# ana-kuznetsova/Policy-Gradient-ASR

Hardware: AMD Instinct MI355X
Metric: utterances/sec (B=32,T=1000,F=80) policy-grad step, 1/2/4/8 MI355X (higher is better)
Workload: dtype f32 (fp32-faithful: fp32 storage and accumulate; every big product -- recurrent sweeps, W_ih projections, input and weight gradients -- on the bf16 MFMA as SIX terms of a 3-plane split hi/mid/lo, every term down to 2^-24 of the product; the small products on the exact fp32 MFMA; the faster bf16x3 mo

## Files before the change

include/pgasr_hip.h:

```cpp
#ifndef PGASR_HIP_H
#define PGASR_HIP_H

#include <stddef.h>
#include <stdint.h>

#ifdef __cplusplus
extern "C" {
#endif

typedef enum pgasr_status {
    PGASR_OK = 0,
    PGASR_ERR_INVALID_ARG = 1,
    PGASR_ERR_LAUNCH = 2,
    PGASR_ERR_WORKSPACE = 3,
    PGASR_ERR_UNSUPPORTED = 4,
    PGASR_ERR_TIMEOUT = 5
} pgasr_status;

#define PGASR_ABI_VERSION 7

int pgasr_abi_version(void);
const char* pgasr_status_string(int status);

size_t pgasr_ctc_workspace_bytes(int T, int B, int V, int Lmax);
int pgasr_ctc_loss_grad(const float* log_probs, const int32_t* targets,
                        const int32_t* input_lengths, const int32_t* target_lengths,
                        int T, int B, int V, int Lmax, int blank,
                        const float* utt_scale, const float* pg_coef, const int32_t* pg_path,
                        float* nll, float* grad_logits,
                        void* workspace, size_t workspace_bytes, void* stream);

int pgasr_ctc_grad_from_lattice(const float* log_probs, const int32_t* input_lengths,
                                const int32_t* target_lengths, int T, int B, int V, int Lmax, int blank,
                                const float* utt_scale, const float* pg_coef, const int32_t* pg_path,
                                int pg_coef_per_frame, float* grad_logits, void* workspace, size_t workspace_bytes,
                                void* stream);

int pgasr_pg_rewards(const int32_t* dist, const int32_t* target_lengths, int B, float lam,
                     float inv_global_batch, float* R_greedy, float* R_sample, float* pg_coef,
                     float* utt_scale, void* stream);
int pgasr_pg_loss_value(const float* log_probs, const int32_t* path, const int32_t* input_lengths,
                        const float* nll, const float* utt_scale, const float* pg_coef,
                        int T, int B, int V, int pg_coef_per_frame, float* terms, void* stream);
int pgasr_pg_step_coefs(const int32_t* paths, const int32_t* input_lengths, const int32_t* prefix_dist, int prefix_stride,
                        const int32_t* token_lengths, const int32_t* target_lengths, int T, int B, int blank,
                        float lam, float inv_global_batch, float* coef, void* stream);

#define PGASR_MAX_SAMPLES 16
#define PGASR_BASELINE_HYPOTHESIS 0
#define PGASR_BASELINE_LEAVE_ONE_OUT 1
int pgasr_frame_sample_multi(const float* scores, int T, int B, int V, int K,
                             uint64_t seed, uint32_t offset, int ctr_stride, int ctr_base,
                             int32_t* greedy_path, int32_t* sample_paths, void* stream);
int pgasr_ctc_grad_from_lattice_multi(const float* log_probs, const int32_t* input_lengths,
                                      const int32_t* target_lengths, int T, int B, int V, int Lmax, int blank,
                                      const float* utt_scale, int K, const float* pg_coef, const int32_t* pg_paths,
                                      float* grad_logits, void* workspace, size_t workspace_bytes, void* stream);
int pgasr_pg_rewards_multi(const int32_t* dist, const int32_t* target_lengths, int B, int K, int baseline,
                           float lam, float inv_global_batch, float* R_baseline, float* R_sample, float* pg_coef,
                           float* utt_scale, void* stream);
int pgasr_pg_loss_value_multi(const float* log_probs, const int32_t* paths, int K, const int32_t* input_lengths,
                              const float* nll, const float* utt_scale, const float* pg_coef,
                              int T, int B, int V, float* terms, void* stream);

size_t pgasr_ctc_hyp_workspace_bytes(int T, int B, int V, int K, int Lh);
int pgasr_ctc_hyp_lattice(const float* log_probs, const int32_t* hyp_tokens, int hyp_stride, const int32_t* hyp_len,
                          const int32_t* input_lengths, int T, int B, int V, int K, int Lh, int blank,
                          float* hyp_nll, void* hyp_workspace, size_t hyp_workspace_bytes, void* stream);
int pgasr_ctc_grad_from_lattices_seq(const float* log_probs, const int32_t* input_lengths, const int32_t* target_lengths,
// ... 180 lines not shown
```

policy_gradient_asr_amd/_lib.py:

```python
import ctypes as C
import os

import torch

_HERE = os.path.dirname(os.path.abspath(__file__))
LIB_PATH = os.environ.get("PGASR_HIP_LIB", os.path.join(_HERE, "libpgasr_hip.so"))

c_f32p = C.c_void_p
c_i32p = C.c_void_p
c_ptr = C.c_void_p

SIGNATURES = {
    "pgasr_abi_version": (C.c_int, []),
    "pgasr_status_string": (C.c_char_p, [C.c_int]),
    "pgasr_ctc_workspace_bytes": (C.c_size_t, [C.c_int, C.c_int, C.c_int, C.c_int]),
    "pgasr_ctc_loss_grad": (C.c_int, [c_f32p, c_i32p, c_i32p, c_i32p, C.c_int, C.c_int, C.c_int, C.c_int,
                                      C.c_int, c_f32p, c_f32p, c_i32p, c_f32p, c_f32p, c_ptr, C.c_size_t, c_ptr]),
    "pgasr_ctc_grad_from_lattice": (C.c_int, [c_f32p, c_i32p, c_i32p, C.c_int, C.c_int, C.c_int, C.c_int, C.c_int,
                                              c_f32p, c_f32p, c_i32p, C.c_int, c_f32p, c_ptr, C.c_size_t, c_ptr]),
    "pgasr_pg_rewards": (C.c_int, [c_i32p, c_i32p, C.c_int, C.c_float, C.c_float, c_f32p, c_f32p, c_f32p, c_f32p, c_ptr]),
    "pgasr_pg_loss_value": (C.c_int, [c_f32p, c_i32p, c_i32p, c_f32p, c_f32p, c_f32p, C.c_int, C.c_int, C.c_int, C.c_int,
                                      c_f32p, c_ptr]),
    "pgasr_head_logsoftmax": (C.c_int, [c_f32p, C.c_longlong, C.c_int, C.c_int, c_f32p, c_f32p, C.c_int, c_f32p, c_f32p, c_ptr]),
    "pgasr_pg_step_coefs": (C.c_int, [c_i32p, c_i32p, c_i32p, C.c_int, c_i32p, c_i32p, C.c_int, C.c_int, C.c_int,
                                      C.c_float, C.c_float, c_f32p, c_ptr]),
    "pgasr_frame_argmax_sample": (C.c_int, [c_f32p, C.c_int, C.c_int, C.c_int, C.c_uint64, C.c_uint32, C.c_int, C.c_int,
                                            c_i32p, c_i32p, c_ptr]),
    "pgasr_frame_sample_multi": (C.c_int, [c_f32p, C.c_int, C.c_int, C.c_int, C.c_int, C.c_uint64, C.c_uint32, C.c_int, C.c_int,
                                           c_i32p, c_i32p, c_ptr]),
    "pgasr_frame_argmax_sample_ids": (C.c_int, [c_f32p, C.c_int, C.c_int, C.c_int, C.c_uint64, C.c_uint32, C.c_int, c_i32p,
                                                c_i32p, c_i32p, c_ptr]),
    "pgasr_frame_sample_multi_ids": (C.c_int, [c_f32p, C.c_int, C.c_int, C.c_int, C.c_int, C.c_uint64, C.c_uint32, C.c_int, c_i32p,
                                               c_i32p, c_i32p, c_ptr]),
    "pgasr_ctc_grad_from_lattice_multi": (C.c_int, [c_f32p, c_i32p, c_i32p, C.c_int, C.c_int, C.c_int, C.c_int, C.c_int,
                                                    c_f32p, C.c_int, c_f32p, c_i32p, c_f32p, c_ptr, C.c_size_t, c_ptr]),
    "pgasr_pg_rewards_multi": (C.c_int, [c_i32p, c_i32p, C.c_int, C.c_int, C.c_int, C.c_float, C.c_float, c_f32p, c_f32p, c_f32p,
                                         c_f32p, c_ptr]),
    "pgasr_pg_loss_value_multi": (C.c_int, [c_f32p, c_i32p, C.c_int, c_i32p, c_f32p, c_f32p, c_f32p, C.c_int, C.c_int, C.c_int,
                                            c_f32p, c_ptr]),
    "pgasr_ctc_hyp_workspace_bytes": (C.c_size_t, [C.c_int] * 5),
    "pgasr_ctc_hyp_lattice": (C.c_int, [c_f32p, c_i32p, C.c_int, c_i32p, c_i32p, C.c_int, C.c_int, C.c_int, C.c_int, C.c_int, C.c_int,
                                        c_f32p, c_ptr, C.c_size_t, c_ptr]),
    "pgasr_ctc_grad_from_lattices_seq": (C.c_int, [c_f32p, c_i32p, c_i32p, C.c_int, C.c_int, C.c_int, C.c_int, C.c_int, c_f32p,
                                                   C.c_int, c_f32p, c_i32p, c_i32p, C.c_int, c_f32p, c_ptr, C.c_size_t,
                                                   c_ptr, C.c_size_t, c_ptr]),
    "pgasr_pg_loss_value_seq": (C.c_int, [c_f32p, c_i32p, C.c_int, c_i32p, c_f32p, c_f32p, c_f32p, c_f32p, c_i32p, C.c_int,
                                          C.c_int, C.c_int, C.c_int, c_f32p, c_ptr]),
    "pgasr_word_ids": (C.c_int, [c_i32p, c_i32p, C.c_int, c_i32p, c_i32p, C.c_int, C.c_int, C.c_int, c_i32p, c_i32p, c_i32p, c_i32p,
                                 c_ptr]),
    "pgasr_pg_rewards_multi_ex": (C.c_int, [c_i32p, c_i32p, c_i32p, C.c_int, C.c_int, C.c_int, C.c_float, C.c_float, c_f32p, c_f32p,
                                            c_f32p, c_f32p, c_ptr]),
    "pgasr_batch_prep": (C.c_int, [c_f32p, C.c_int, C.c_int, c_ptr, c_ptr, C.c_int, c_i32p, c_i32p, c_i32p, c_ptr]),
# ... 118 lines not shown
```

policy_gradient_asr_amd/csrc/ctc.hip:

```cpp
#include "common.h"

namespace {

constexpr int CTC_THREADS = 256;
constexpr int CTC_SPT = 8;
constexpr int CTC_SMAX = CTC_THREADS * CTC_SPT;
constexpr int CTC_VMAX = 64;

struct CtcWs {
    float* alpha;
    float* beta;
    int SP;
    double* amax;
    double* bmax;
    double* nll64;
    int32_t* lab_off;
    int32_t* lab_states;
};

__host__ __device__ inline size_t ctc_ws_layout(int T, int B, int V, int Smax, CtcWs* ws, char* base) {
    size_t off = 0;
    auto take = [&](size_t bytes) { size_t o = off; off += (bytes + 255) / 256 * 256; return o; };
    const int SP = (Smax + 63) / 64 * 64;
    size_t a = take((size_t)B * T * SP * sizeof(float));
// ... 246 lines not shown
            }
            occ = acc;
        }
        const float sc = utt_scale ? utt_scale[b] : 1.f;
        g = sc * (sm - occ);
    }
    return g;
}

__global__ __launch_bounds__(256) void ctc_grad_kernel(
    const float* __restrict__ lp, const int32_t* __restrict__ in_len, const int32_t* __restrict__ tg_len,
    int T, int B, int V, int Lmax, int Smax, int blank, CtcWs ws,
    const float* __restrict__ utt_scale, const float* __restrict__ pg_coef,
    const int32_t* __restrict__ pg_path, int coef_per_frame, float* __restrict__ grad) {
    const int lane = threadIdx.x & 63;
    const long long w = (long long)blockIdx.x * (blockDim.x >> 6) + (threadIdx.x >> 6);
    if (w >= (long long)T * B) return;
    const int t = (int)(w / B), b = (int)(w % B);
    int Tb = in_len[b]; Tb = Tb < 0 ? 0 : (Tb > T ? T : Tb);
    int Lb = tg_len[b]; Lb = Lb < 0 ? 0 : (Lb > Lmax ? Lmax : Lb);
    const size_t o = ((size_t)t * B + b) * V;
    if (t >= Tb) { if (lane < V) grad[o + lane] = 0.f; return; }

    const float lpv = (lane < V) ? lp[o + lane] : 0.f;
    const float sm = (lane < V) ? __expf(lpv) : 0.f;
    float g = ctc_grad_row(lpv, sm, lane, t, b, T, V, Lb, Smax, blank, ws, utt_scale);
    if (pg_coef != nullptr && pg_path != nullptr) {
        const int k = pg_path[(size_t)t * B + b];
        g += pg_coef[coef_per_frame ? (size_t)t * B + b : (size_t)b] * (sm - (lane == k ? 1.f : 0.f));
    }
    if (lane < V) grad[o + lane] = g;
}

__global__ __launch_bounds__(256) void ctc_grad_multi_kernel(
    const float* __restrict__ lp, const int32_t* __restrict__ in_len, const int32_t* __restrict__ tg_len,
    int T, int B, int V, int Lmax, int Smax, int blank, CtcWs ws,
    const float* __restrict__ utt_scale, int K, const float* __restrict__ pg_coef,
    const int32_t* __restrict__ pg_paths, float* __restrict__ grad) {
    const int lane = threadIdx.x & 63;
    const long long w = (long long)blockIdx.x * (blockDim.x >> 6) + (threadIdx.x >> 6);
    if (w >= (long long)T * B) return;
    const int t = (int)(w / B), b = (int)(w % B);
    int Tb = in_len[b]; Tb = Tb < 0 ? 0 : (Tb > T ? T : Tb);
    int Lb = tg_len[b]; Lb = Lb < 0 ? 0 : (Lb > Lmax ? Lmax : Lb);
    const size_t o = ((size_t)t * B + b) * V;
    if (t >= Tb) { if (lane < V) grad[o + lane] = 0.f; return; }

    const float lpv = (lane < V) ? lp[o + lane] : 0.f;
    const float sm = (lane < V) ? __expf(lpv) : 0.f;
    float g = ctc_grad_row(lpv, sm, lane, t, b, T, V, Lb, Smax, blank, ws, utt_scale);
    const size_t TB = (size_t)T * B;
    for (int k = 0; k < K; ++k) {
        const int pk = pg_paths[k * TB + (size_t)t * B + b];
        g += pg_coef[(size_t)k * B + b] * (sm - (lane == pk ? 1.f : 0.f));
    }
    if (lane < V) grad[o + lane] = g;
}


template <int NMAX>
__global__ __launch_bounds__(CTC_THREADS + 64) void ctc_hyp_lattice_kernel(
    const float* __restrict__ lp, const int32_t* __restrict__ hyp, int hyp_stride, const int32_t* __restrict__ hyp_len,
    const int32_t* __restrict__ in_len, int T, int B, int V, int Lh, int Smax, int blank, CtcWs ws, float* __restrict__ hyp_nll) {
    __shared__ double rows[2 * (NMAX * CTC_THREADS + 4)];
    const int p = blockIdx.x, b = p % B, role = blockIdx.y;
    const int len = hyp_len[p];
// ... 130 lines not shown
    if (ok != PGASR_OK) return ok;
    const int Smax = 2 * Lmax + 1;
    CtcWs ws;
    if (!ctc_ws_bind(T, B, V, Smax, &ws, workspace, workspace_bytes)) return PGASR_ERR_WORKSPACE;
    hipStream_t st = (hipStream_t)stream;
#define PGASR_LATTICE(NSPT) PGASR_LAUNCH_KERNEL(ctc_lattice_kernel<NSPT>, dim3(B, 3), dim3(CTC_THREADS + 64), 0, st, \
                        log_probs, targets, input_lengths, target_lengths, T, B, V, Lmax > 0 ? Lmax : 1, Smax, blank, ws, nll, 0)
    if (Smax <= CTC_THREADS) PGASR_LATTICE(1);
    else if (Smax <= 2 * CTC_THREADS) PGASR_LATTICE(2);
    else if (Smax <= 4 * CTC_THREADS) PGASR_LATTICE(4);
    else PGASR_LATTICE(8);
#undef PGASR_LATTICE
    PGASR_CHECK_LAUNCH();
    if (!grad_logits) return PGASR_OK;
    return ctc_launch_grad(ctc_grad_kernel, log_probs, input_lengths, target_lengths, T, B, V, Lmax, blank, ws, utt_scale, stream,
                           pg_coef, pg_path, 0, grad_logits);
}

extern "C" int pgasr_ctc_grad_from_lattice(const float* log_probs, const int32_t* input_lengths,
                                           const int32_t* target_lengths, int T, int B, int V, int Lmax, int blank,
                                           const float* utt_scale, const float* pg_coef, const int32_t* pg_path,
                                           int pg_coef_per_frame, float* grad_logits, void* workspace, size_t workspace_bytes,
                                           void* stream) {
    if (!log_probs || !input_lengths || !target_lengths || !grad_logits) return PGASR_ERR_INVALID_ARG;
    if ((pg_coef == nullptr) != (pg_path == nullptr)) return PGASR_ERR_INVALID_ARG;
    const int ok = ctc_args_ok(T, B, V, Lmax, blank);
    if (ok != PGASR_OK) return ok;
    CtcWs ws;
    if (!ctc_ws_bind(T, B, V, 2 * Lmax + 1, &ws, workspace, workspace_bytes)) return PGASR_ERR_WORKSPACE;
    return ctc_launch_grad(ctc_grad_kernel, log_probs, input_lengths, target_lengths, T, B, V, Lmax, blank, ws, utt_scale, stream,
                           pg_coef, pg_path, pg_coef_per_frame ? 1 : 0, grad_logits);
}

extern "C" int pgasr_ctc_grad_from_lattice_multi(const float* log_probs, const int32_t* input_lengths,
                                                 const int32_t* target_lengths, int T, int B, int V, int Lmax, int blank,
                                                 const float* utt_scale, int K, const float* pg_coef, const int32_t* pg_paths,
                                                 float* grad_logits, void* workspace, size_t workspace_bytes, void* stream) {
    if (!log_probs || !input_lengths || !target_lengths || !grad_logits || !pg_coef || !pg_paths) return PGASR_ERR_INVALID_ARG;
    if (K < 1 || K > PGASR_MAX_SAMPLES) return PGASR_ERR_INVALID_ARG;
    const int ok = ctc_args_ok(T, B, V, Lmax, blank);
    if (ok != PGASR_OK) return ok;
    CtcWs ws;
    if (!ctc_ws_bind(T, B, V, 2 * Lmax + 1, &ws, workspace, workspace_bytes)) return PGASR_ERR_WORKSPACE;
    return ctc_launch_grad(ctc_grad_multi_kernel, log_probs, input_lengths, target_lengths, T, B, V, Lmax, blank, ws, utt_scale, stream,
                           K, pg_coef, pg_paths, grad_logits);
}

extern "C" size_t pgasr_ctc_hyp_workspace_bytes(int T, int B, int V, int K, int Lh) {
    if (ctc_hyp_args_ok(T, B, V, K, Lh) != PGASR_OK) return 0;
    return ctc_ws_layout(T, K * B, V, 2 * Lh + 1, nullptr, nullptr);
}

extern "C" int pgasr_ctc_hyp_lattice(const float* log_probs, const int32_t* hyp_tokens, int hyp_stride, const int32_t* hyp_len,
                                     const int32_t* input_lengths, int T, int B, int V, int K, int Lh, int blank,
                                     float* hyp_nll, void* hyp_workspace, size_t hyp_workspace_bytes, void* stream) {
    if (!log_probs || !hyp_tokens || !hyp_len || !input_lengths || !hyp_nll) return PGASR_ERR_INVALID_ARG;
    if (blank < 0 || blank >= V || hyp_stride < 1 || hyp_stride < Lh) return PGASR_ERR_INVALID_ARG;
    const int ok = ctc_hyp_args_ok(T, B, V, K, Lh);
    if (ok != PGASR_OK) return ok;
    const int Smax = 2 * Lh + 1;
    CtcWs ws;
    if (!ctc_ws_bind(T, K * B, V, Smax, &ws, hyp_workspace, hyp_workspace_bytes)) return PGASR_ERR_WORKSPACE;
    hipStream_t st = (hipStream_t)stream;
#define PGASR_HYP_LATTICE(NMAX) PGASR_LAUNCH_KERNEL(ctc_hyp_lattice_kernel<NMAX>, dim3(K * B, 3), dim3(CTC_THREADS + 64), 0, st, \
                        log_probs, hyp_tokens, hyp_stride, hyp_len, input_lengths, T, B, V, Lh, Smax, blank, ws, hyp_nll)
    if (Smax <= CTC_THREADS) PGASR_HYP_LATTICE(1);
// ... 40 lines not shown
```

policy_gradient_asr_amd/functional.py:

```python
import os

import torch

from . import hipops
from . import streams

HID = hipops.HID
FEED_AHEAD = os.environ.get("PGASR_FEED_AHEAD", "1") != "0"
JOIN_FEED = os.environ.get("PGASR_JOIN_FEED", "0") == "1"
FEED_BWD = os.environ.get("PGASR_FEED_BWD", "1") != "0"
STREAM_DW = os.environ.get("PGASR_STREAM_DW", "1") != "0"
LEAKY_SLOPE = 0.01


def _pick_splitk(M, N, K, target_wgs=512, batch=1, beside_sweep=False):
    if M % 256 == 0 and N % 256 == 0 and K % 32 == 0 and K >= 64:
        tiles = (M // 256) * (N // 256) * batch
        sk = max(1, min((128 if beside_sweep else 256) // tiles, K // 256))
        while sk > 1 and (sk - 1) * (-(-K // sk // 32) * 32) >= K:
            sk -= 1
        return sk
    tiles = ((M + 127) // 128) * ((N + 127) // 128)
    sk = max(1, min(64, target_wgs // max(tiles, 1)))
    while sk > 1 and K // sk < 256:
# ... 169 lines not shown
        ctx.nopt = len(opt)
        if ctx.fused:
            ctx.save_for_backward(x)
        return hipops.dropout(x, p, seed, offset)

    @staticmethod
    def backward(ctx, dy):
        p, seed, offset = ctx.cfg
        rec = grad_overlap._deferred.get(dy.data_ptr())
        if rec is not None and not ctx.fused and rec["drop"] is None and dy.shape == rec["dx"].shape:
            rec["drop"] = (p, seed, offset)
            return (dy, None, None, None) + (None,) * ctx.nopt
        dact = ctx.saved_tensors[0] if ctx.fused else None
        return (hipops.dropout(dy.contiguous(), p, seed, offset, dact_y=dact, slope=LEAKY_SLOPE), None, None, None) + (None,) * ctx.nopt


class LinearFn(torch.autograd.Function):

    @staticmethod
    def forward(ctx, x, weight, bias):
        shp = x.shape
        x2 = x.contiguous().view(-1, shp[-1])
        rows, K = x2.shape
        N = weight.shape[0]
        weight = weight.contiguous()
        y = torch.empty(rows, N, dtype=torch.float32, device=x.device)
        hipops.gemm(x2, weight, y, M=rows, N=N, K=K, transB=True, bias=bias.contiguous())
        ctx.save_for_backward(x2, weight)
        ctx.shp = shp
        ctx.param_refs = (weight, bias)
        return y.view(*shp[:-1], N)

    @staticmethod
    def backward(ctx, dy):
        x2, weight = ctx.saved_tensors
        rows, K = x2.shape
        N = weight.shape[0]
        dy2 = dy.contiguous().view(rows, N)
        dx = torch.empty(rows, K, dtype=torch.float32, device=dy.device)
        hipops.gemm(dy2, weight, dx, M=rows, N=K, K=N)
        wg, bg = (p.grad for p in ctx.param_refs)
        if grad_overlap.enabled and wg is not None and bg is not None and wg.is_contiguous() and bg.is_contiguous():
            done = torch.cuda.Event()
            done.record()
            grad_overlap.note_event(done)

            def weight_grads():
                hipops.gemm(dy2, x2, wg, M=N, N=K, K=rows, transA=True, lda=N, splitk=_pick_splitk(N, K, rows), accumulate=True)
                hipops.colsum(dy2, rows, N, N, bg, accumulate=True)
            grad_overlap.pending().append((done, weight_grads))
            side = grad_overlap.side_stream()
            streams.hold(dy2, side); streams.hold(x2, side)
            return dx.view(ctx.shp), None, None
        dW = torch.empty(N, K, dtype=torch.float32, device=dy.device)
        hipops.gemm(dy2, x2, dW, M=N, N=K, K=rows, transA=True, lda=N, splitk=_pick_splitk(N, K, rows))
        db = torch.empty(N, dtype=torch.float32, device=dy.device)
        hipops.colsum(dy2, rows, N, N, db)
        return dx.view(ctx.shp), dW, db


class HeadFn(torch.autograd.Function):

    @staticmethod
    def forward(ctx, x, weight, bias):
        shp = x.shape
        x2 = x.contiguous().view(-1, shp[-1])
        weight = weight.contiguous()
        logits, lp = hipops.head_logsoftmax(x2, weight, bias.contiguous())
        ctx.save_for_backward(x2, weight)
        ctx.shp = shp
        ctx.param_refs = (weight, bias)
        lp = lp.view(*shp[:-1], -1)
        ctx.mark_non_differentiable(lp)
        return logits.view(*shp[:-1], -1), lp

    @staticmethod
    def backward(ctx, dy, _dlp=None):
        return LinearFn.backward(ctx, dy)


class LogSoftmaxFn(torch.autograd.Function):
    @staticmethod
    def forward(ctx, logits):
        lp = hipops.log_softmax_rows(logits.contiguous())
        ctx.save_for_backward(lp)
        return lp

    @staticmethod
    def backward(ctx, g):
        (lp,) = ctx.saved_tensors
        return g - torch.exp(lp) * g.sum(dim=-1, keepdim=True)


class BLSTMLayerFn(torch.autograd.Function):

    @staticmethod
    def forward(ctx, x, lengths, dact_y, sweep_follows, prepacked, out_dropout, w_ih_f, w_hh_f, b_ih_f, b_hh_f, w_ih_r, w_hh_r, b_ih_r, b_hh_r):
        T, B, I = x.shape
        x = x.contiguous()
        if prepacked is None:
            prepacked = prepack_blstm((w_ih_f, w_hh_f, b_ih_f, b_hh_f, w_ih_r, w_hh_r, b_ih_r, b_hh_r), I)
        elif prepacked.ready is not None:
            torch.cuda.current_stream().wait_event(prepacked.ready)
        wih_perm, bias_perm, pack_f, pack_b = prepacked.wih_perm, prepacked.bias_perm, prepacked.pack_f, prepacked.pack_b
        ctx.planes_t = prepacked.planes_t
        npl = len(prepacked.planes) if prepacked.planes is not None else hipops.LSTM_PLANES
        ctx.nplanes = npl
        ctx.fed_bwd = prepacked.fed_bwd
        prepacked.fed_bwd = None
        ctx.slab_words = prepacked.slab
        prepacked.slab = None
# ... 281 lines not shown
```

policy_gradient_asr_amd/hipops.py:

```python
import os

import torch

_os_environ_get = os.environ.get

from . import _lib


def _stream():
    return torch.cuda.current_stream().cuda_stream


def _req(t, dtype, name):
    if t is None:
        return None
    if not t.is_cuda:
        raise _lib.PgasrError(f"{name} must live on the GPU (got {t.device}); there is no CPU path")
    if t.dtype != dtype:
        raise _lib.PgasrError(f"{name} must be {dtype} (got {t.dtype})")
    if not t.is_contiguous():
        raise _lib.PgasrError(f"{name} must be contiguous")
    return t


# ... 122 lines not shown
    return 1


def _grad_pass(entry, log_probs, input_lengths, target_lengths, handle, utt_scale, pg_coef, paths, paths_name, mid, ws_tail=(),
               label=None):
    lib = _lib.load()
    ws, Lmax, blank = handle
    T, B, V = log_probs.shape
    _req(utt_scale, torch.float32, "utt_scale"); _req(pg_coef, torch.float32, "pg_coef"); _req(paths, torch.int32, paths_name)
    grad = torch.empty_like(log_probs)
    with _timed(label):
        st = getattr(lib, entry)(_p(log_probs), _p(input_lengths), _p(target_lengths), T, B, V, Lmax, blank, _p(utt_scale),
                                 *(a if isinstance(a, int) else _p(a) for a in mid), _p(grad), _p(ws), ws.numel(), *ws_tail, _stream())
    _lib.check(st, entry)
    return grad


def _loss_value(entry, log_probs, paths, paths_name, input_lengths, nll, utt_scale, pg_coef, K=(), mid=(), tail=()):
    lib = _lib.load()
    T, B, V = log_probs.shape
    _req(log_probs, torch.float32, "log_probs"); _req(paths, torch.int32, paths_name); _req(nll, torch.float32, "nll")
    _req(utt_scale, torch.float32, "utt_scale"); _req(pg_coef, torch.float32, "pg_coef")
    terms = torch.empty(B, dtype=torch.float32, device=log_probs.device)
    st = getattr(lib, entry)(_p(log_probs), _p(paths), *K, _p(input_lengths), _p(nll), _p(utt_scale), _p(pg_coef), *mid,
                             T, B, V, *tail, _p(terms), _stream())
    _lib.check(st, entry)
    return terms


def ctc_grad_from_lattice(log_probs, input_lengths, target_lengths, handle, utt_scale=None, pg_coef=None, pg_path=None):
    T, B, _ = log_probs.shape
    return _grad_pass("pgasr_ctc_grad_from_lattice", log_probs, input_lengths, target_lengths, handle, utt_scale, pg_coef, pg_path,
                      "pg_path", (pg_coef, pg_path, _coef_per_frame(pg_coef, T, B)))


def pg_rewards(dist, target_lengths, lam, inv_global_batch):
    lib = _lib.load()
    _req(dist, torch.int32, "dist"); _req(target_lengths, torch.int32, "target_lengths")
    B = target_lengths.numel()
    if dist.numel() != 2 * B:
        raise _lib.PgasrError("pg_rewards wants 2*B distances")
    out = torch.empty(4, B, dtype=torch.float32, device=dist.device)
    st = lib.pgasr_pg_rewards(_p(dist), _p(target_lengths), B, float(lam), float(inv_global_batch),
                              out[0].data_ptr(), out[1].data_ptr(), out[2].data_ptr(), out[3].data_ptr(), _stream())
    _lib.check(st, "pgasr_pg_rewards")
    return out[0], out[1], out[2], out[3]


def pg_loss_value(log_probs, path, input_lengths, nll, utt_scale, pg_coef):
    T, B, _ = log_probs.shape
    return _loss_value("pgasr_pg_loss_value", log_probs, path, "path", input_lengths, nll, utt_scale, pg_coef,
                       tail=(_coef_per_frame(pg_coef, T, B),))


MAX_SAMPLES = 16
BASELINES = {"hypothesis": 0, "leave_one_out": 1}


def ctc_grad_from_lattice_multi(log_probs, input_lengths, target_lengths, handle, utt_scale, pg_coef, pg_paths):
    T, B, _ = log_probs.shape
    K = pg_paths.shape[0]
    if pg_paths.dim() != 3 or tuple(pg_paths.shape[1:]) != (T, B) or tuple(pg_coef.shape) != (K, B):
        raise _lib.PgasrError(f"ctc_grad_from_lattice_multi wants pg_paths (K,{T},{B}) and pg_coef (K,{B})")
    return _grad_pass("pgasr_ctc_grad_from_lattice_multi", log_probs, input_lengths, target_lengths, handle, utt_scale, pg_coef,
                      pg_paths, "pg_paths", (K, pg_coef, pg_paths))

# ... 839 lines not shown
```

policy_gradient_asr_amd/loss.py:

```python
import dataclasses
import numbers

import torch
import torch.nn as nn

from . import hipops
from . import streams


class customNLLLoss(nn.Module):

    def __init__(self, ignore_index=None):
        super().__init__()
        self.ignore_index = ignore_index

    def forward(self, inp, target):
        L, B, V = inp.shape
        tgt = target.t().unsqueeze(-1).long()
        picked = -inp.gather(2, tgt).squeeze(-1)
        if self.ignore_index:
            keep = (target.t() != self.ignore_index).to(inp.dtype)
            return ((picked * keep).sum(dim=1) / keep.sum(dim=1)).sum()
        return picked.mean(dim=1).sum()


class PGCTCLossFn(torch.autograd.Function):

    _lattice_streams = {}
    unit_seed_ptr = None
    unit_hits = 0
    last_sequence_scored = None
    @staticmethod
    def forward(ctx, logits, in_len, targets, tg_len, log_probs, sample_ids, opt):
        T, B, V = logits.shape
        PGCTCLossFn.last_sequence_scored = None
        K, beam, blank = opt.num_samples, opt.beam, opt.blank
        loo = opt.baseline == "leave_one_out"
        wd = opt.word_delimiter if opt.reward_unit == "word" else None
        Lh = hipops.hyp_len_cap(T, opt.max_hyp_len) if opt.score_function == "sequence" else None
        single = K == 1 and not loo and Lh is None
        greedy_row = not loo and beam == 0
        P = K + (0 if loo else 1)
        inv_gb = 1.0 / float(opt.global_batch)
        dev = logits.device
        lp = log_probs
        if lp is None or lp.shape != logits.shape or not lp.is_contiguous():
            lp = hipops.log_softmax_rows(logits.contiguous())
        main = torch.cuda.current_stream()
        side = PGCTCLossFn._lattice_streams.setdefault(main.cuda_stream, None) or streams.side_stream("loss_section")
        PGCTCLossFn._lattice_streams[main.cuda_stream] = side
        if sample_ids is not None:
            lay = {"batch_stride": opt.global_batch, "utt_ids": sample_ids}
        else:
            lay = {"batch_stride": opt.global_batch, "batch_offset": opt.sample_base} if opt.sample_base >= 0 else {}
        side.wait_stream(main)
        with torch.cuda.stream(side):
            if single:
                greedy, sample = hipops.frame_argmax_sample(lp, seed=opt.seed, offset=opt.offset, want_greedy=greedy_row, **lay)
                samples = sample[None]
                paths = torch.stack((greedy, sample), dim=0) if greedy_row else samples
            elif greedy_row:
                paths = torch.empty(P, T, B, dtype=torch.int32, device=dev)
                hipops.frame_sample_multi(lp, K, seed=opt.seed, offset=opt.offset, out=(paths[0], paths[1:]), **lay)
                samples = paths[1:]
            else:
                _, samples = hipops.frame_sample_multi(lp, K, seed=opt.seed, offset=opt.offset, **lay)
                paths = samples
            if beam > 0 and not loo:
                tokens = torch.zeros(P, B, T, dtype=torch.int32, device=dev)
                tok_len = torch.empty(P, B, dtype=torch.int32, device=dev)
                hipops.ctc_beam_search(lp, in_len, beam=beam, blank=blank, collapse=True, out=(tokens[0], tok_len[0]))
                hipops.ctc_collapse(samples, in_len, blank=blank, out=(tokens[1:], tok_len[1:]))
            else:
                tokens, tok_len = hipops.ctc_collapse(paths, in_len, blank=blank)
            if Lh is not None:
                hyp_len = tok_len[P - K:]
                hyp_nll, hyp_lattice = hipops.ctc_hyp_lattice(lp, tokens[P - K:], hyp_len, in_len, Lh, blank=blank)
                PGCTCLossFn.last_sequence_scored = scored = hyp_len <= Lh
            n_words = prefix = None
            if wd is not None:
                dist, n_words = _word_distances(targets, tg_len, tokens, tok_len, P, wd)
            else:
                dist = hipops.edit_distance(targets.repeat(P, 1), tg_len.repeat(P), tokens.view(P * B, T), tok_len.view(P * B),
                                            want_prefix=opt.per_step)
                if opt.per_step:
                    dist, prefix = dist
            if single and wd is None:
                R_b, R_s, coef, utt_scale = hipops.pg_rewards(dist, tg_len, opt.lam, inv_gb)
            else:
                R_b, R_s, coef, utt_scale = hipops.pg_rewards_multi(dist, tg_len, K, opt.lam, inv_gb, baseline=opt.baseline,
                                                                    reward_lengths=n_words)
                if single:
                    R_s, coef = R_s[0], coef[0]
            if opt.per_step:
                coef = hipops.pg_step_coefs(paths, in_len, prefix, tok_len.view(2 * B), tg_len, opt.lam, inv_gb, blank=blank)
        nll, lattice = hipops.ctc_lattice(lp, targets, in_len, tg_len, blank=blank)
        main.wait_stream(side)
        for t_ in (samples, R_b, R_s, coef, utt_scale) + ((tok_len, hyp_nll, scored) if Lh is not None else ()):
            streams.hold(t_, main)
        if single:
            grad = hipops.ctc_grad_from_lattice(lp, in_len, tg_len, lattice, utt_scale=utt_scale, pg_coef=coef, pg_path=sample)
            loss = hipops.pg_loss_value(lp, sample, in_len, nll, utt_scale, coef).sum()
        elif Lh is None:
            grad = hipops.ctc_grad_from_lattice_multi(lp, in_len, tg_len, lattice, utt_scale, coef, samples)
            loss = hipops.pg_loss_value_multi(lp, samples, in_len, nll, utt_scale, coef).sum()
        else:
            grad = hipops.ctc_grad_from_lattices_seq(lp, in_len, tg_len, lattice, hyp_lattice, utt_scale, coef, samples, hyp_len)
            loss = hipops.pg_loss_value_seq(lp, samples, in_len, nll, utt_scale, coef, hyp_nll, hyp_len, Lh).sum()
        ctx.save_for_backward(grad)
        ctx.mark_non_differentiable(nll, R_s, R_b)
        ctx.set_materialize_grads(False)
        return loss, nll, R_s, R_b

    @staticmethod
    def backward(ctx, g, *unused):
        (grad,) = ctx.saved_tensors
        if PGCTCLossFn.unit_seed_ptr is not None and g.data_ptr() == PGCTCLossFn.unit_seed_ptr and g.numel() == 1:
            PGCTCLossFn.unit_hits += 1
        else:
            grad = grad * g
        return (grad,) + (None,) * (len(ctx.needs_input_grad) - 1)


REWARD_UNITS = ("char", "word")


def _word_distances(targets, tg_len, tokens, tok_len, P, delimiter):
    B, T = tokens.shape[1], tokens.shape[2]
    dist, ref_words, _ = hipops.word_edit_distance(targets.repeat(P, 1), tg_len.repeat(P), tokens.view(P * B, T),
                                                   tok_len.view(P * B), delimiter)
    return dist, ref_words[:B]


@dataclasses.dataclass(frozen=True)
class PGOptions:
    lam: float = 1.0
    seed: int = 0
    offset: int = 0
    global_batch: int = 1
    blank: int = 0
    beam: int = 0
    sample_base: int = -1
    per_step: bool = False
    num_samples: int = 1
    baseline: str = "hypothesis"
    reward_unit: str = "char"
    word_delimiter: object = None
    score_function: str = "path"
    max_hyp_len: object = None


# ... 39 lines not shown
            raise ValueError("max_hyp_len caps the hypotheses that score_function='sequence' scores: it has no meaning with 'path'")
    if score_function == "sequence" and per_step:
        raise ValueError("per-step rewards have frame-aligned coefficients, which have no sequence form: score_function='sequence' "
                         "does not take reward_mode='per_step'")


def _check_samples(num_samples, baseline, per_step=False):
    if baseline not in hipops.BASELINES:
        raise ValueError(f"baseline must be one of {sorted(hipops.BASELINES)} (got {baseline!r})")
    if isinstance(num_samples, bool) or int(num_samples) != num_samples:
        raise ValueError(f"num_samples must be an integer (got {num_samples!r})")
    if not 1 <= num_samples <= hipops.MAX_SAMPLES:
        raise ValueError(f"num_samples {num_samples} outside 1 .. {hipops.MAX_SAMPLES}: the multi-sample kernels take at most "
                         f"{hipops.MAX_SAMPLES} paths per utterance")
    if baseline == "leave_one_out" and num_samples < 2:
        raise ValueError("the leave-one-out baseline needs num_samples >= 2 (the other samples' rewards)")
    if per_step and num_samples > 1:
        raise ValueError("per-step rewards take one sampled path (num_samples = 1)")


def pg_ctc_loss(logits, in_len, targets, tg_len, lam=1.0, seed=0, offset=0, global_batch=None, blank=0, beam=0, sample_base=-1,
                per_step=False, log_probs=None, num_samples=1, baseline="hypothesis", reward_unit="char", word_delimiter=None,
                sample_ids=None, score_function="path", max_hyp_len=None):
    T, B, V = logits.shape
    opt = check_options(PGOptions(lam=float(lam), seed=int(seed), offset=int(offset), global_batch=int(global_batch or B),
                                  blank=int(blank), beam=int(beam), sample_base=int(sample_base), per_step=bool(per_step),
                                  num_samples=num_samples, baseline=baseline, reward_unit=reward_unit, word_delimiter=word_delimiter,
                                  score_function=score_function, max_hyp_len=max_hyp_len),
                        vocab=V, frames=T, symbols=targets.shape[1] if targets.dim() == 2 else 0, sample_ids=sample_ids)
    if log_probs is None:
        log_probs = getattr(logits, "log_probs", None)
        if log_probs is not None and getattr(logits, "log_probs_version", None) != logits._version:
            log_probs = None
    return PGCTCLossFn.apply(logits, in_len, targets, tg_len, log_probs, sample_ids, opt)


class CTCLoss(nn.Module):

    def __init__(self, blank=0):
        super().__init__()
        self.blank = blank

    def forward(self, logits, in_len, targets, tg_len, global_batch=None):
        loss, _, _, _ = pg_ctc_loss(logits, in_len, targets, tg_len, lam=0.0, global_batch=global_batch,
                                    blank=self.blank)
        return loss
```

policy_gradient_asr_amd/model.py:

```python
import torch
import torch.nn as nn

from . import functional as Fh
from . import hipops
from . import streams

HID = 256


def weights(m):
    if isinstance(m, nn.Linear):
        nn.init.xavier_normal_(m.weight.data)
        nn.init.constant_(m.bias.data, 0.1)


def nan_to_num(t, mynan=0.):
    if torch.all(torch.isfinite(t)):
        return t
    return torch.where(torch.isfinite(t), t, torch.as_tensor(mynan, dtype=t.dtype, device=t.device))


class Encoder(nn.Module):

    def __init__(self, n_feats=120):
# ... 66 lines not shown
        H = self.hidden_size
        w_ih, w_hh = self.lstm.weight_ih_l0.detach().contiguous(), self.lstm.weight_hh_l0.detach().contiguous()
        bias = (self.lstm.bias_ih_l0 + self.lstm.bias_hh_l0).detach().contiguous()
        if not w_ih.is_cuda:
            raise RuntimeError("Decoder.forward runs on the MI355X only (no CPU path)")
        B, L = target_inputs.shape
        x = self.embed_layer.weight.detach()[target_inputs.to(w_ih.device)].transpose(0, 1).contiguous()
        xp = torch.empty(L * B, 4 * H, dtype=torch.float32, device=w_ih.device)
        hipops.gemm(x.view(L * B, 128), w_ih, xp, M=L * B, N=4 * H, K=128, transB=True, bias=bias, precision=0)
        xp = xp.view(L, B, 4 * H)
        h = torch.zeros(B, H, dtype=torch.float32, device=w_ih.device)
        c = torch.zeros_like(h)
        g = torch.empty(B, 4 * H, dtype=torch.float32, device=w_ih.device)
        dec_out = torch.empty(L, B, H, dtype=torch.float32, device=w_ih.device)
        for t in range(L):
            hipops.gemm(h, w_hh, g, M=B, N=4 * H, K=H, transB=True, precision=0)
            hipops.lstm_cell(g, xp[t], c, h, dec_out[t])
        ctx = hipops.attention_ctx(dec_out, encoder_outputs.to(w_ih.device).contiguous())
        return torch.cat((dec_out, ctx), dim=2)


class Seq2Seq(nn.Module):

    def __init__(self, alphabet_size, n_feats=120):
        super().__init__()
        self.encoder = Encoder(n_feats=n_feats)
        self.head = nn.Linear(2 * HID, alphabet_size)

    def logits(self, x, fmask, lengths=None):
        h, lengths = self.encoder.forward_time_major(x, fmask, lengths)
        if hipops.head_logsoftmax_ok(self.head.in_features, self.head.out_features):
            z, lp = Fh.HeadFn.apply(h, self.head.weight, self.head.bias)
            z.log_probs = lp
            z.log_probs_version = z._version
            return z, lengths
        return Fh.LinearFn.apply(h, self.head.weight, self.head.bias), lengths

    def forward(self, x, t, fmask, device=None):
        z, _ = self.logits(x, fmask)
        return Fh.LogSoftmaxFn.apply(z)


def _read_alphabet(alphabet_path):
    with open(alphabet_path, "r") as fo:
        alphabet = ["<pad>"] + fo.readlines()
    char2ind = {alphabet[i].replace("\n", ""): i for i in range(len(alphabet))}
    return alphabet, char2ind


def _to_device(batch, device):
    x = batch["feat"].to(device)
    t = batch["trans"].to(device)
    fmask = batch["fmask"].squeeze(1).to(device)
    tmask = batch["tmask"].squeeze(1).to(device)
    return x, t, fmask, tmask


FEATURE_DIMS = {"mfcc": 120, "logmel80": 80}


def _check_features(features, n_feats, dataset):
    if features not in FEATURE_DIMS:
        raise ValueError(f"features must be one of {sorted(FEATURE_DIMS)}")
    try:
        item = dataset[0] if dataset is not None and len(dataset) > 0 else None
    except Exception:
# ... 179 lines not shown
```

policy_gradient_asr_amd/train_step.py:

```python
import os
import threading

import torch
import torch.distributed as dist

FLAG_PAD = 64
_step_lock = threading.Lock()


def flatten_parameters(model, pad=0):
    params = [p for p in model.parameters()]
    dev = params[0].device
    total = pad + sum(p.numel() for p in params)
    flat = torch.zeros(total, dtype=torch.float32, device=dev)
    gflat = torch.zeros(total, dtype=torch.float32, device=dev)
    off = pad
    with torch.no_grad():
        for p in params:
            n = p.numel()
            flat[off:off + n].copy_(p.data.view(-1))
            p.data = flat[off:off + n].view_as(p.data)
            p.grad = gflat[off:off + n].view_as(p.data)
            off += n
    return flat, gflat
# ... 364 lines not shown
        if side is None:
            from . import streams
            side = streams.side_stream("loss_section")
            PGCTCLossFn._lattice_streams[main.cuda_stream] = side
        return side

    def _upper_grads_issued(self, swept):
        from .functional import grad_overlap
        side = grad_overlap.side_stream()
        s3 = grad_overlap._sides3.get(grad_overlap._key()) if grad_overlap._streamed_unjoined.get(grad_overlap._key()) else None
        with torch.cuda.stream(side):
            side.wait_event(swept)
            if s3 is not None:
                side.wait_stream(s3)
            self.reduce_upper(self.upper_split)

    def backward(self, loss):
        from .functional import grad_overlap
        from .loss import PGCTCLossFn
        grad_overlap.enabled = self.overlap_weight_grads
        early = (self.collective and self.early_reduce and self.overlap_weight_grads and self.upper_split is not None
                 and not self._hold_collectives)
        grad_overlap.upper_grads_hook = self._upper_grads_issued if early else None
        if self._one is None or self._one.device != loss.device:
            self._one = torch.ones((), dtype=loss.dtype, device=loss.device)
        PGCTCLossFn.unit_seed_ptr = self._one.data_ptr()
        try:
            loss.backward(gradient=self._one)
        except BaseException:
            grad_overlap._deferred.clear()
            raise
        finally:
            PGCTCLossFn.unit_seed_ptr = None
            grad_overlap.enabled = False
            grad_overlap.upper_grads_hook = None
            grad_overlap.finish()

    def _padded(self, x, targets, fmask, tmask):
        from . import hipops
        B = x.shape[0]
        q = 16 if hipops.LSTM_PLANES == 3 else 32
        Bp = -(-B // q) * q
        if not (self.pad_ragged_batches and x.is_cuda and Bp != B and Bp <= 32 and targets.dim() == 2 and fmask.dim() == 2):
            return x, targets, fmask, tmask
        n = Bp - B
        grow = lambda t_: torch.cat((t_, t_.new_zeros((n,) + tuple(t_.shape[1:]))), dim=0)
        return grow(x), grow(targets), grow(fmask), grow(tmask)

    def forward_loss(self, batch, global_batch):
        from .loss import PGCTCLossFn, pg_ctc_loss
        x, targets, fmask, tmask = batch
        from . import hipops
        self._check_limits(x, targets)
        real_b = x.shape[0]
        x, targets, fmask, tmask = self._padded(x, targets, fmask, tmask)
        padded = x.shape[0] != real_b
        if (fmask.dtype == torch.float32 and tmask.dtype == torch.int64 and targets.dtype == torch.int64 and targets.dim() == 2
                and targets.shape[1] > 0 and fmask.is_contiguous() and tmask.is_contiguous() and targets.is_contiguous()):
            in_len, tg_len, tg = hipops.batch_prep(fmask, tmask, targets)
        else:
            in_len = None
            tg_len = tmask.sum(dim=1).to(torch.int32).contiguous()
            tg = targets.to(torch.int32).contiguous()
        logits, in_len = self.model.logits(x, fmask, in_len)
        sample_base, sample_ids = self._sample_addressing(real_b, x.shape[0], x.device)
        loss, nll, R_s, R_g = pg_ctc_loss(logits, in_len, tg, tg_len, lam=self.lam, seed=self.seed,
                                          offset=self.nstep + 1, global_batch=global_batch, blank=self.blank,
                                          beam=self.beam_size if self.reward_decoder == "beam" else 0,
                                          sample_base=sample_base,
                                          per_step=self.reward_mode == "per_step", num_samples=self.num_samples,
                                          baseline=self.reward_baseline, reward_unit=self.reward_unit,
                                          word_delimiter=self.word_delimiter, sample_ids=sample_ids,
                                          score_function=self.score_function, max_hyp_len=self.max_hyp_len)
        scored = PGCTCLossFn.last_sequence_scored
        self.last_sequence_scored = scored[:, :real_b] if (padded and scored is not None) else scored
        R_all = R_s if R_s.dim() == 2 else R_s.view(1, -1)
        if R_s.dim() == 2:
            R_s = R_s.mean(dim=0)
        self.last_sample_rewards = R_all[:, :real_b] if padded else R_all
        self.last_stats = (nll[:real_b], R_s[:real_b], R_g[:real_b]) if padded else (nll, R_s, R_g)
        if self._micro is not None and self._micro.count > 1:
            self._micro_stats.append((self.last_stats, self.last_sample_rewards, self.last_sequence_scored))
        return loss

    def _sample_addressing(self, real_b, padded_b, device):
        mb = self._micro
        n_micro = mb.count if mb is not None else 1
        padded = padded_b != real_b
        if mb is not None and mb.ids is not None:
            host = torch.tensor(mb.ids + [-1] * (padded_b - real_b), dtype=torch.int32)
            if device.type == "cuda":
                host = host.pin_memory()
            return -1, host.to(device, non_blocking=True)
        base = self.world * (mb.offset if mb is not None else 0) + self.rank * real_b
        if padded and (self.world > 1 or n_micro > 1):
            ids = torch.arange(base, base + padded_b, dtype=torch.int32, device=device)
            ids[real_b:] = -1
            return -1, ids
        return (base if (self.world > 1 or padded or n_micro > 1) else -1), None

    def _accumulate(self, micro_batches, utt_ids, hold_last=False):
        self._micro_stats = []
        try:
            loss = super()._accumulate(micro_batches, utt_ids, hold_last=hold_last)
            if len(self._micro_stats) > 1:
                self.last_stats = tuple(torch.cat([st[i] for st, _, _ in self._micro_stats]) for i in range(3))
# ... 7 lines not shown
```

Baseline: 3370.

## Fuse CTC logit gradient with head input-gradient GEMM and defer loss value

Adds a kernel that computes the CTC/policy-gradient logit gradient rows and, in the same block, multiplies them by the head weight on the fp32 MFMA to produce the encoder gradient. The result is parked and reused by HeadFn.backward so the separate dx GEMM is skipped. The loss-value reduction is also moved onto a side stream and joined at the end of the step. This removes a kernel launch and a round trip of the gradient through memory. In exchange it adds global parking state keyed by pointers, with fallbacks when version or shape checks fail.

Result: no change. 3363 (median of 2 runs) (-0.2%).

```diff
diff --git a/include/pgasr_hip.h b/include/pgasr_hip.h
--- a/include/pgasr_hip.h
+++ b/include/pgasr_hip.h
@@ -35,6 +35,12 @@
                                 const float* utt_scale, const float* pg_coef, const int32_t* pg_path,
                                 int pg_coef_per_frame, float* grad_logits, void* workspace, size_t workspace_bytes,
                                 void* stream);
+
+int pgasr_ctc_grad_denc_from_lattice(const float* log_probs, const int32_t* input_lengths,
+                                     const int32_t* target_lengths, int T, int B, int V, int Lmax, int blank,
+                                     const float* utt_scale, const float* pg_coef, const int32_t* pg_path,
+                                     int pg_coef_per_frame, float* grad_logits, void* workspace, size_t workspace_bytes,
+                                     const float* head_weight, int hidden, float* d_enc, void* stream);
 
 int pgasr_pg_rewards(const int32_t* dist, const int32_t* target_lengths, int B, float lam,
                      float inv_global_batch, float* R_greedy, float* R_sample, float* pg_coef,
diff --git a/policy_gradient_asr_amd/_lib.py b/policy_gradient_asr_amd/_lib.py
--- a/policy_gradient_asr_amd/_lib.py
+++ b/policy_gradient_asr_amd/_lib.py
@@ -18,6 +18,9 @@
                                       C.c_int, c_f32p, c_f32p, c_i32p, c_f32p, c_f32p, c_ptr, C.c_size_t, c_ptr]),
     "pgasr_ctc_grad_from_lattice": (C.c_int, [c_f32p, c_i32p, c_i32p, C.c_int, C.c_int, C.c_int, C.c_int, C.c_int,
                                               c_f32p, c_f32p, c_i32p, C.c_int, c_f32p, c_ptr, C.c_size_t, c_ptr]),
+    "pgasr_ctc_grad_denc_from_lattice": (C.c_int, [c_f32p, c_i32p, c_i32p, C.c_int, C.c_int, C.c_int, C.c_int, C.c_int,
+                                                   c_f32p, c_f32p, c_i32p, C.c_int, c_f32p, c_ptr, C.c_size_t,
+                                                   c_f32p, C.c_int, c_f32p, c_ptr]),
     "pgasr_pg_rewards": (C.c_int, [c_i32p, c_i32p, C.c_int, C.c_float, C.c_float, c_f32p, c_f32p, c_f32p, c_f32p, c_ptr]),
     "pgasr_pg_loss_value": (C.c_int, [c_f32p, c_i32p, c_i32p, c_f32p, c_f32p, c_f32p, C.c_int, C.c_int, C.c_int, C.c_int,
                                       c_f32p, c_ptr]),
diff --git a/policy_gradient_asr_amd/csrc/ctc.hip b/policy_gradient_asr_amd/csrc/ctc.hip
--- a/policy_gradient_asr_amd/csrc/ctc.hip
+++ b/policy_gradient_asr_amd/csrc/ctc.hip
@@ -302,6 +302,69 @@
     if (lane < V) grad[o + lane] = g;
 }
 
+constexpr int DENC_ROWS = 32, DENC_N = 512;
+typedef __attribute__((ext_vector_type(16))) float ctc_f32x16;
+__global__ __launch_bounds__(512) void ctc_grad_denc_kernel(
+    const float* __restrict__ lp, const int32_t* __restrict__ in_len, const int32_t* __restrict__ tg_len,
+    int T, int B, int V, int Lmax, int Smax, int blank, CtcWs ws,
+    const float* __restrict__ utt_scale, const float* __restrict__ pg_coef,
+    const int32_t* __restrict__ pg_path, int coef_per_frame, float* __restrict__ grad,
+    const float* __restrict__ w_head, float* __restrict__ denc) {
+    __shared__ float tile[DENC_ROWS][DENC_ROWS + 1];
+    const int lane = threadIdx.x & 63, wv = threadIdx.x >> 6;
+    const int cl = lane & 31, kh = lane >> 5;
+    const long long rows = (long long)T * B;
+    const long long row0 = (long long)blockIdx.x * DENC_ROWS;
+    const int kend = (V + 15) / 16 * 16;
+    for (int i = 0; i < 4; ++i) {
+        const int r = wv * 4 + i;
+        const long long w = row0 + r;
+        float g = 0.f;
+        if (w < rows) {
+            const int t = (int)(w / B), b = (int)(w % B);
+            int Tb = in_len[b]; Tb = Tb < 0 ? 0 : (Tb > T ? T : Tb);
+            int Lb = tg_len[b]; Lb = Lb < 0 ? 0 : (Lb > Lmax ? Lmax : Lb);
+            const size_t o = ((size_t)t * B + b) * V;
+            if (t < Tb) {
+                const float lpv = (lane < V) ? lp[o + lane] : 0.f;
+                const float sm = (lane < V) ? __expf(lpv) : 0.f;
+                g = ctc_grad_row(lpv, sm, lane, t, b, T, V, Lb, Smax, blank, ws, utt_scale);
+                if (pg_coef != nullptr && pg_path != nullptr) {
+                    const int k = pg_path[(size_t)t * B + b];
+                    g += pg_coef[coef_per_frame ? (size_t)t * B + b : (size_t)b] * (sm - (lane == k ? 1.f : 0.f));
+                }
+            }
+            if (lane < V) grad[o + lane] = g;
+        }
+        if (lane < DENC_ROWS) tile[r][lane] = lane < V ? g : 0.f;
+    }
+    __syncthreads();
+    const long long live = rows - row0 < DENC_ROWS ? rows - row0 : DENC_ROWS;
+    __amdgpu_buffer_rsrc_t drs = __builtin_amdgcn_make_buffer_rsrc(denc + (size_t)row0 * DENC_N, 0, (int)(live * DENC_N * 4), 0x00020000);
+#pragma unroll 1
+    for (int j = 0; j < 2; ++j) {
+        const int col = wv * 64 + j * 32 + cl;
+        float wb[16];
+#pragma unroll
+        for (int s = 0; s < 16; ++s) {
+            const int k = 2 * s + kh;
+            wb[s] = k < V ? w_head[(size_t)k * DENC_N + col] : 0.f;
+        }
+        ctc_f32x16 acc;
+#pragma unroll
+        for (int e = 0; e < 16; ++e) acc[e] = 0.f;
+#pragma unroll
+        for (int s = 0; s < 16; ++s)
+            if (2 * s < kend) acc = __builtin_amdgcn_mfma_f32_32x32x2f32(tile[cl][2 * s + kh], wb[s], acc, 0, 0, 0);
+        const unsigned o0 = (unsigned)(((4 * kh) * DENC_N + col) * 4);
+#pragma unroll
+        for (int e = 0; e < 16; ++e) {
+            const float v = 1.f * acc[e] + 0.f;
+            __builtin_amdgcn_raw_buffer_store_b32(__float_as_uint(v), drs, o0 + (unsigned)(((e & 3) + 8 * (e >> 2)) * DENC_N * 4), 0, 0);
+        }
+    }
+}
+
 __global__ __launch_bounds__(256) void ctc_grad_multi_kernel(
     const float* __restrict__ lp, const int32_t* __restrict__ in_len, const int32_t* __restrict__ tg_len,
     int T, int B, int V, int Lmax, int Smax, int blank, CtcWs ws,
@@ -498,6 +561,28 @@
                            pg_coef, pg_path, pg_coef_per_frame ? 1 : 0, grad_logits);
 }
 
+extern "C" int pgasr_ctc_grad_denc_from_lattice(const float* log_probs, const int32_t* input_lengths,
+                                                const int32_t* target_lengths, int T, int B, int V, int Lmax, int blank,
+                                                const float* utt_scale, const float* pg_coef, const int32_t* pg_path,
+                                                int pg_coef_per_frame, float* grad_logits, void* workspace, size_t workspace_bytes,
+                                                const float* head_weight, int hidden, float* d_enc, void* stream) {
+    if (!log_probs || !input_lengths || !target_lengths || !grad_logits || !head_weight || !d_enc) return PGASR_ERR_INVALID_ARG;
+    if ((pg_coef == nullptr) != (pg_path == nullptr)) return PGASR_ERR_INVALID_ARG;
+    const int ok = ctc_args_ok(T, B, V, Lmax, blank);
+    if (ok != PGASR_OK) return ok;
+    if (V > DENC_ROWS || hidden != DENC_N) return PGASR_ERR_UNSUPPORTED;
+    CtcWs ws;
+    if (!ctc_ws_bind(T, B, V, 2 * Lmax + 1, &ws, workspace, workspace_bytes)) return PGASR_ERR_WORKSPACE;
+    const long long rows = (long long)T * B;
+    const long long blocks = (rows + DENC_ROWS - 1) / DENC_ROWS;
+    if (blocks > 0x7fffffffLL) return PGASR_ERR_UNSUPPORTED;
+    PGASR_LAUNCH_KERNEL(ctc_grad_denc_kernel, dim3((unsigned)blocks), dim3(512), 0, (hipStream_t)stream,
+                       log_probs, input_lengths, target_lengths, T, B, V, Lmax > 0 ? Lmax : 1, 2 * Lmax + 1, blank, ws, utt_scale,
+                       pg_coef, pg_path, pg_coef_per_frame ? 1 : 0, grad_logits, head_weight, d_enc);
+    PGASR_CHECK_LAUNCH();
+    return PGASR_OK;
+}
+
 extern "C" int pgasr_ctc_grad_from_lattice_multi(const float* log_probs, const int32_t* input_lengths,
                                                  const int32_t* target_lengths, int T, int B, int V, int Lmax, int blank,
                                                  const float* utt_scale, int K, const float* pg_coef, const int32_t* pg_paths,
diff --git a/policy_gradient_asr_amd/functional.py b/policy_gradient_asr_amd/functional.py
--- a/policy_gradient_asr_amd/functional.py
+++ b/policy_gradient_asr_amd/functional.py
@@ -225,13 +225,14 @@
         return y.view(*shp[:-1], N)
 
     @staticmethod
-    def backward(ctx, dy):
+    def backward(ctx, dy, dx=None):
         x2, weight = ctx.saved_tensors
         rows, K = x2.shape
         N = weight.shape[0]
         dy2 = dy.contiguous().view(rows, N)
-        dx = torch.empty(rows, K, dtype=torch.float32, device=dy.device)
-        hipops.gemm(dy2, weight, dx, M=rows, N=K, K=N)
+        if dx is None:
+            dx = torch.empty(rows, K, dtype=torch.float32, device=dy.device)
+            hipops.gemm(dy2, weight, dx, M=rows, N=K, K=N)
         wg, bg = (p.grad for p in ctx.param_refs)
         if grad_overlap.enabled and wg is not None and bg is not None and wg.is_contiguous() and bg.is_contiguous():
             done = torch.cuda.Event()
@@ -269,7 +270,16 @@
 
     @staticmethod
     def backward(ctx, dy, _dlp=None):
-        return LinearFn.backward(ctx, dy)
+        from .loss import PGCTCLossFn
+        dx = None
+        rec = PGCTCLossFn._parked.pop(dy.data_ptr(), None) if PGCTCLossFn._parked else None
+        if rec is not None:
+            grad, d_enc, w_ptr, w_version = rec
+            weight = ctx.saved_tensors[1]
+            if (hipops.GEMM_PRECISION == 0 and dy.is_contiguous() and dy.numel() == grad.numel() and weight.data_ptr() == w_ptr
+                    and weight._version == w_version and tuple(d_enc.shape) == (ctx.saved_tensors[0].shape[0], weight.shape[1])):
+                dx = d_enc
+        return LinearFn.backward(ctx, dy, dx)
 
 
 class LogSoftmaxFn(torch.autograd.Function):
diff --git a/policy_gradient_asr_amd/hipops.py b/policy_gradient_asr_amd/hipops.py
--- a/policy_gradient_asr_amd/hipops.py
+++ b/policy_gradient_asr_amd/hipops.py
@@ -178,6 +178,28 @@
     T, B, _ = log_probs.shape
     return _grad_pass("pgasr_ctc_grad_from_lattice", log_probs, input_lengths, target_lengths, handle, utt_scale, pg_coef, pg_path,
                       "pg_path", (pg_coef, pg_path, _coef_per_frame(pg_coef, T, B)))
+
+
+CHAIN_FUSIONS = _os_environ_get("PGASR_CHAIN_FUSIONS", "1") != "0"
+GRAD_DENC_MAX_V, GRAD_DENC_HIDDEN = 32, 512
+
+
+def ctc_grad_denc_ok(log_probs, head_weight):
+    V = log_probs.shape[-1]
+    return (GEMM_PRECISION == 0 and head_weight is not None and head_weight.is_cuda and head_weight.dtype == torch.float32
+            and head_weight.is_contiguous() and tuple(head_weight.shape) == (V, GRAD_DENC_HIDDEN) and V <= GRAD_DENC_MAX_V)
+
+
+def ctc_grad_denc_from_lattice(log_probs, input_lengths, target_lengths, handle, head_weight, utt_scale=None, pg_coef=None, pg_path=None):
+    T, B, _ = log_probs.shape
+    _req(head_weight, torch.float32, "head_weight")
+    if not ctc_grad_denc_ok(log_probs, head_weight):
+        raise _lib.PgasrError("ctc_grad_denc_from_lattice: head_weight must be (V, 512) fp32 with V <= 32, in the exact-fp32 GEMM mode")
+    d_enc = torch.empty(T * B, GRAD_DENC_HIDDEN, dtype=torch.float32, device=log_probs.device)
+    grad = _grad_pass("pgasr_ctc_grad_denc_from_lattice", log_probs, input_lengths, target_lengths, handle, utt_scale, pg_coef, pg_path,
+                      "pg_path", (pg_coef, pg_path, _coef_per_frame(pg_coef, T, B)),
+                      ws_tail=(_p(head_weight), GRAD_DENC_HIDDEN, _p(d_enc)))
+    return grad, d_enc
 
 
 def pg_rewards(dist, target_lengths, lam, inv_global_batch):
diff --git a/policy_gradient_asr_amd/loss.py b/policy_gradient_asr_amd/loss.py
--- a/policy_gradient_asr_amd/loss.py
+++ b/policy_gradient_asr_amd/loss.py
@@ -30,8 +30,12 @@
     unit_seed_ptr = None
     unit_hits = 0
     last_sequence_scored = None
+    _parked = {}
+    fuse_head_grad = False
+    defer_value = False
+    _value_unjoined = {}
     @staticmethod
-    def forward(ctx, logits, in_len, targets, tg_len, log_probs, sample_ids, opt):
+    def forward(ctx, logits, in_len, targets, tg_len, log_probs, sample_ids, opt, head_weight=None):
         T, B, V = logits.shape
         PGCTCLossFn.last_sequence_scored = None
         K, beam, blank = opt.num_samples, opt.beam, opt.blank
@@ -98,7 +102,25 @@
         main.wait_stream(side)
         for t_ in (samples, R_b, R_s, coef, utt_scale) + ((tok_len, hyp_nll, scored) if Lh is not None else ()):
             streams.hold(t_, main)
-        if single:
+        ctx.d_enc = None
+        if single and hipops.CHAIN_FUSIONS:
+            if PGCTCLossFn.fuse_head_grad and ctx.needs_input_grad[0] and hipops.ctc_grad_denc_ok(lp, head_weight):
+                grad, d_enc = hipops.ctc_grad_denc_from_lattice(lp, in_len, tg_len, lattice, head_weight, utt_scale=utt_scale,
+                                                                pg_coef=coef, pg_path=sample)
+                ctx.d_enc = (d_enc, head_weight.data_ptr(), head_weight._version)
+            else:
+                grad = hipops.ctc_grad_from_lattice(lp, in_len, tg_len, lattice, utt_scale=utt_scale, pg_coef=coef, pg_path=sample)
+            if PGCTCLossFn.defer_value:
+                latticed = torch.cuda.Event()
+                latticed.record()
+                with torch.cuda.stream(side):
+                    side.wait_event(latticed)
+                    loss = hipops.pg_loss_value(lp, sample, in_len, nll, utt_scale, coef).sum()
+                streams.hold(lp, side); streams.hold(nll, side); streams.hold(loss, main)
+                PGCTCLossFn._value_unjoined[main.cuda_stream] = side
+            else:
+                loss = hipops.pg_loss_value(lp, sample, in_len, nll, utt_scale, coef).sum()
+        elif single:
             grad = hipops.ctc_grad_from_lattice(lp, in_len, tg_len, lattice, utt_scale=utt_scale, pg_coef=coef, pg_path=sample)
             loss = hipops.pg_loss_value(lp, sample, in_len, nll, utt_scale, coef).sum()
         elif Lh is None:
@@ -115,8 +137,11 @@
     @staticmethod
     def backward(ctx, g, *unused):
         (grad,) = ctx.saved_tensors
+        PGCTCLossFn._parked.clear()
         if PGCTCLossFn.unit_seed_ptr is not None and g.data_ptr() == PGCTCLossFn.unit_seed_ptr and g.numel() == 1:
             PGCTCLossFn.unit_hits += 1
+            if ctx.d_enc is not None:
+                PGCTCLossFn._parked[grad.data_ptr()] = (grad,) + ctx.d_enc
         else:
             grad = grad * g
         return (grad,) + (None,) * (len(ctx.needs_input_grad) - 1)
@@ -222,7 +247,10 @@
         log_probs = getattr(logits, "log_probs", None)
         if log_probs is not None and getattr(logits, "log_probs_version", None) != logits._version:
             log_probs = None
-    return PGCTCLossFn.apply(logits, in_len, targets, tg_len, log_probs, sample_ids, opt)
+    head_weight = getattr(logits, "head_weight", None)
+    if head_weight is not None and getattr(logits, "log_probs_version", None) != logits._version:
+        head_weight = None
+    return PGCTCLossFn.apply(logits, in_len, targets, tg_len, log_probs, sample_ids, opt, head_weight)
 
 
 class CTCLoss(nn.Module):
diff --git a/policy_gradient_asr_amd/model.py b/policy_gradient_asr_amd/model.py
--- a/policy_gradient_asr_amd/model.py
+++ b/policy_gradient_asr_amd/model.py
@@ -122,6 +122,7 @@
         if hipops.head_logsoftmax_ok(self.head.in_features, self.head.out_features):
             z, lp = Fh.HeadFn.apply(h, self.head.weight, self.head.bias)
             z.log_probs = lp
+            z.head_weight = self.head.weight.detach()
             z.log_probs_version = z._version
             return z, lengths
         return Fh.LinearFn.apply(h, self.head.weight, self.head.bias), lengths
diff --git a/policy_gradient_asr_amd/train_step.py b/policy_gradient_asr_amd/train_step.py
--- a/policy_gradient_asr_amd/train_step.py
+++ b/policy_gradient_asr_amd/train_step.py
@@ -420,6 +420,10 @@
             raise
         finally:
             PGCTCLossFn.unit_seed_ptr = None
+            PGCTCLossFn._parked.clear()
+            value_side = PGCTCLossFn._value_unjoined.pop(torch.cuda.current_stream().cuda_stream, None)
+            if value_side is not None:
+                torch.cuda.current_stream().wait_stream(value_side)
             grad_overlap.enabled = False
             grad_overlap.upper_grads_hook = None
             grad_overlap.finish()
@@ -452,14 +456,19 @@
             tg = targets.to(torch.int32).contiguous()
         logits, in_len = self.model.logits(x, fmask, in_len)
         sample_base, sample_ids = self._sample_addressing(real_b, x.shape[0], x.device)
-        loss, nll, R_s, R_g = pg_ctc_loss(logits, in_len, tg, tg_len, lam=self.lam, seed=self.seed,
-                                          offset=self.nstep + 1, global_batch=global_batch, blank=self.blank,
-                                          beam=self.beam_size if self.reward_decoder == "beam" else 0,
-                                          sample_base=sample_base,
-                                          per_step=self.reward_mode == "per_step", num_samples=self.num_samples,
-                                          baseline=self.reward_baseline, reward_unit=self.reward_unit,
-                                          word_delimiter=self.word_delimiter, sample_ids=sample_ids,
-                                          score_function=self.score_function, max_hyp_len=self.max_hyp_len)
+        PGCTCLossFn.defer_value = x.is_cuda and type(self).forward_loss is PolicyGradientTrainer.forward_loss
+        PGCTCLossFn.fuse_head_grad = x.is_cuda
+        try:
+            loss, nll, R_s, R_g = pg_ctc_loss(logits, in_len, tg, tg_len, lam=self.lam, seed=self.seed,
+                                              offset=self.nstep + 1, global_batch=global_batch, blank=self.blank,
+                                              beam=self.beam_size if self.reward_decoder == "beam" else 0,
+                                              sample_base=sample_base,
+                                              per_step=self.reward_mode == "per_step", num_samples=self.num_samples,
+                                              baseline=self.reward_baseline, reward_unit=self.reward_unit,
+                                              word_delimiter=self.word_delimiter, sample_ids=sample_ids,
+                                              score_function=self.score_function, max_hyp_len=self.max_hyp_len)
+        finally:
+            PGCTCLossFn.defer_value = PGCTCLossFn.fuse_head_grad = False
         scored = PGCTCLossFn.last_sequence_scored
         self.last_sequence_scored = scored[:, :real_b] if (padded and scored is not None) else scored
         R_all = R_s if R_s.dim() == 2 else R_s.view(1, -1)
```
